# AlainSchoebi/semantic-bundle-adjustment-colmap

Measured on AMD Instinct MI355X. Metric: residuals+Jacobians/sec and BA-iteration wall-time, 1k cams / 1M pts / 10M obs, higher is better.
Workload: dtype f64

## Files before the change

semantic-bundle-adjustment-colmap_amd/csrc/context.h:

```cpp
#pragma once

#include <hip/hip_runtime.h>
#include <rocblas/rocblas.h>
#include <rccl/rccl.h>

#include <map>
#include <string>
#include <vector>

#include "../../include/mi_ba.h"
#include "cholesky.h"
#include "device.h"
#include "setup.h"

namespace miba {

template <typename T>
struct DevArray {
  T* ptr = nullptr;
  size_t n = 0;
  size_t cap = 0;
  DevArray() = default;
  DevArray(const DevArray&) = delete;
  DevArray& operator=(const DevArray&) = delete;
// ... 67 lines not shown
  int lin_overlap = 0;
  int lin_warm = 15;
  int lin_warm_conc = 0;
  int warm_unroll = 4;
  int warm_wgs = 2048;
  int lin_order = 0;
  int lin_fusion = 1;
  hipStream_t lin_side = nullptr;
  hipEvent_t lin_ev[2] = {nullptr, nullptr};
  int sem_diag = 0;
  bool sem_deferred_box = false;
  int sem_prep_early = 0;
  int sem_dgrid = 24;
  bool sem_dgrid_set = false;
  int sem_dwaves = 4;
  int sem_dvar = 0;
  int sem_compact = 1;
  int sem_coarse = 2;
  int sem_variant = 6;

  miba::DevArray<double2> r;
  miba::DevArray<double> J;
  miba::DevArray<double> Jcm;
  bool jcm_stale = true;
  miba::DevArray<double> Vg;
  miba::DevArray<double> partial;
  int64_t npartial = 0;
  miba::DevArray<double> scale_p, diag_p, Vinv;
  miba::DevArray<double> pose_blk, cam_blk, bvec, udiag;
  miba::DevArray<double> scale_f, diag_f, lambda_f, prec_pose, prec_cam;
// ... 84 lines not shown
```

semantic-bundle-adjustment-colmap_amd/csrc/runtime.hip:

```cpp
#include <hip/hip_runtime.h>

#include <algorithm>
#include <atomic>
#include <chrono>
#include <condition_variable>
#include <memory>
#include <mutex>
#include <thread>
#include <cmath>
#include <cstdio>
#include <cstring>
#include <cstdlib>
#include <map>
#include <numeric>
#include <unordered_map>

#include "../../include/mi_ba.h"
#include "ba_math.h"
#include "cholesky.h"
#include "context.h"
#include "kernels.h"
#include "gsba.h"
#include "semantic.h"
#include "setup.h"
// ... 2117 lines not shown
    return MI_BA_OK;
  }
  if (std::strcmp(key, "semantic_prep_early") == 0 && (value == 0 || value == 1) && ab_value(value, 0)) {
    ctx->sem_prep_early = value;
    return MI_BA_OK;
  }
  if (std::strcmp(key, "semantic_deferred_variant") == 0 && value >= 0 && value <= 4 && ab_value(value, 0)) {
    ctx->sem_dvar = value;
    return MI_BA_OK;
  }
  if (std::strcmp(key, "semantic_deferred_grid") == 0 && value >= 1 && value <= 64) {
    ctx->sem_dgrid = value;
    ctx->sem_dgrid_set = true;
    return MI_BA_OK;
  }
  if (std::strcmp(key, "semantic_deferred_waves") == 0 && (value == 1 || value == 4)) {
    ctx->sem_dwaves = value;
    return MI_BA_OK;
  }
  if (std::strcmp(key, "linearize_fusion") == 0 && value >= 0 && value <= 7) {
    ctx->lin_fusion = value;
    return MI_BA_OK;
  }
  if (std::strcmp(key, "semantic_deferred_compact") == 0 && (value == 0 || value == 1)) {
    ctx->sem_compact = value;
    return MI_BA_OK;
  }
  if (std::strcmp(key, "semantic_flat_coarse") == 0 && value >= 0 && value <= 3) {
    ctx->sem_coarse = value;
    return MI_BA_OK;
// ... 334 lines not shown
```

semantic-bundle-adjustment-colmap_amd/csrc/semantic.h:

```cpp
#pragma once

#include <hip/hip_runtime.h>

#include <cstdint>
#include <functional>

#include "../../include/mi_ba.h"
#include "ba_math.h"
#include "context.h"

namespace miba {

struct SemSample {
  double pc1[3];
  float label1;
  uint32_t pair;
};

struct SemTile {
  uint32_t pair, start, count, pad;
};

struct SemPair {
  uint32_t i, j;
// ... 35 lines not shown
  DevArray<double> r;
  DevArray<int32_t> status;
  DevArray<double> J;
  DevArray<double> pconst;
  bool samples_valid = false;
  DevArray<double> pair_blk;
  DevArray<double> partial;
  int64_t npartial = 0;
  DevArray<SemTile> tiles;
  int ntiles = 0;
  int model_tiles[kNumModels + 1] = {};
  DevArray<uint32_t> pair_cnt;
  DevArray<uint32_t> dlist;
  DevArray<uint2> chunks;
  DevArray<uint2> dchunks;
  DevArray<uint32_t> dcount;
  DevArray<uint32_t> model_pairs;
  DevArray<uint4> pair_ord;
  bool order_compact = false;
  int n_cu = 256;
  int dwaves_blocks[kNumModels] = {};
  int model_chunks[kNumModels + 1] = {};
  DevArray<unsigned long long> dmask;
  DevArray<uint32_t> pair_tile0, pair_chunk0;
  DevArray<double> cpart;
  DevArray<uint32_t> img_pairs_off, img_pairs;
  DevArray<uint2> sblk;
  DevArray<uint32_t> sblk_off, sblk_ent;
  int nsblk = 0;
  DevArray<double> mpart;
};

mi_ba_status semantic_create(mi_ba_context* ctx, const mi_ba_semantic* sem);
void semantic_destroy(mi_ba_context* ctx);
mi_ba_status semantic_linearize(mi_ba_context* ctx, double* d_cost, bool write_samples,
                                hipStream_t deferred_stream = nullptr, hipEvent_t flat_done = nullptr,
// ... 21 lines not shown
```

semantic-bundle-adjustment-colmap_amd/csrc/semantic.hip:

```cpp
#include <hip/hip_runtime.h>

#include <map>

#include <algorithm>
#include <cmath>
#include <cstring>
#include <type_traits>

#include "ba_math.h"
#include "kernels.h"
#include "semantic.h"
#include "step_bodies.h"

namespace miba {

namespace {

constexpr double kMinStep = 1.4901161193847656e-08;

struct SemArgs {
  const SemSample* samples;
  const SemPair* pairs;
  const double* qt;
  const double* cam;
// ... 310 lines not shown
  const int m = e >> 1;
  const bool minus = e & 1;
  const int grp = m < 4 ? 0 : (m < 7 ? 1 : (m < 11 ? 2 : 3));
  const int k = m - (grp == 0 ? 0 : (grp == 1 ? 4 : (grp == 2 ? 7 : 11)));
  const double orig = grp == 0 ? q1[k] : (grp == 1 ? t1[k] : (grp == 2 ? q2[k] : t2[k]));
  const double delta = fmax(kMinStep, fabs(orig) * rel_step);
  const double pert = minus ? orig - delta : orig + delta;
  P->pert[e] = pert;
  if (minus) {
    double one_over_delta = 1.0 / delta;
    one_over_delta /= 2;
    P->ood[m] = one_over_delta;
  }
  if (grp == 1 || grp == 3) return;
  const double* q = grp == 0 ? q1 : q2;
  double qq[4] = {q[0], q[1], q[2], q[3]};
  qq[k] = pert;
  double Q[9];
  quat_matrix_un(qq, Q);
  const double in = 1.0 / (qq[0] * qq[0] + qq[1] * qq[1] + qq[2] * qq[2] + qq[3] * qq[3]);
  double* A = P->A[grp == 0 ? e : e - 6];
  if (grp == 0) {
    double u2[4], R2[9];
    unit_quat(q2, u2);
    unit_quat_matrix(u2, R2);
    for (int r = 0; r < 3; ++r)
      for (int j = 0; j < 3; ++j)
        A[3 * r + j] = (R2[3 * r] * Q[3 * j] + R2[3 * r + 1] * Q[3 * j + 1] + R2[3 * r + 2] * Q[3 * j + 2]) * in;
  } else {
    for (int c = 0; c < 9; ++c) A[c] = Q[c] * in;
  }
  if (minus) {
    double PJ[12];
    quat_plus_jacobian(q, PJ);
    for (int c = 0; c < 3; ++c) P->pj[(grp == 0 ? 0 : 4) + k][c] = PJ[3 * k + c];
  }
}

constexpr int kPairVals = 78 + 12;
constexpr int kPairStride = 96;
constexpr int kSemRow = 13;

__device__ inline void pair_prep_body(int k, int lane, const SemPair* __restrict__ pairs, int npairs,
                                      const double* __restrict__ qt, const double* __restrict__ cam,
                                      const uint32_t* __restrict__ img_cam, const uint32_t* __restrict__ img_flags,
                                      const uint32_t* __restrict__ raster_slot, const SlotInfo* __restrict__ slots,
                                      double rel_step, PairConst* __restrict__ out, double* __restrict__ pair_blk,
                                      int blk_stride, uint32_t* __restrict__ pair_cnt) {
  if (k >= npairs) return;
  for (int e = lane; e < blk_stride; e += 32) pair_blk[(size_t)k * blk_stride + e] = 0.0;
  if (pair_cnt && lane == 31) pair_cnt[k] = 0u;
  if (lane > 28) return;
  const SemPair pr = pairs[k];
  if (lane < 28) {
    const double* a1 = qt + 8 * (size_t)pr.i;
    const double* a2 = qt + 8 * (size_t)pr.j;
    const double q1[4] = {a1[0], a1[1], a1[2], a1[3]}, t1[3] = {a1[4], a1[5], a1[6]};
    const double q2[4] = {a2[0], a2[1], a2[2], a2[3]}, t2[3] = {a2[4], a2[5], a2[6]};
    stencil_prep(q1, t1, q2, t2, rel_step, lane, out + k);
    return;
  }
  PairConst& P = out[k];
  const double* a1 = qt + 8 * (size_t)pr.i;
  const double* a2 = qt + 8 * (size_t)pr.j;
  for (int m = 0; m < 4; ++m) { P.q1[m] = a1[m]; P.q2[m] = a2[m]; }
  for (int m = 0; m < 3; ++m) { P.t1[m] = a1[4 + m]; P.t2[m] = a2[4 + m]; }
  Pose1Stage s;
  const double zero[3] = {0.0, 0.0, 0.0};
  pose1_stage(P.q1, zero, s);
  {
    const double* q1 = P.q1;
    const double sc = 1.0 / sqrt(q1[0] * q1[0] + q1[1] * q1[1] + q1[2] * q1[2] + q1[3] * q1[3]);
    const double qi[4] = {sc * q1[0], -(sc * q1[1]), -(sc * q1[2]), -(sc * q1[3])};
    const double scale = 1.0 / sqrt(qi[0] * qi[0] + qi[1] * qi[1] + qi[2] * qi[2] + qi[3] * qi[3]);
    for (int m = 0; m < 4; ++m) P.uqi[m] = scale * qi[m];
  }
  P.ti[0] = -(s.R[0] * P.t1[0] + s.R[1] * P.t1[1] + s.R[2] * P.t1[2]);
  P.ti[1] = -(s.R[3] * P.t1[0] + s.R[4] * P.t1[1] + s.R[5] * P.t1[2]);
  P.ti[2] = -(s.R[6] * P.t1[0] + s.R[7] * P.t1[1] + s.R[8] * P.t1[2]);
  unit_quat(P.q2, P.u2);
  unit_quat_matrix(P.u2, P.R2);
  for (int r = 0; r < 3; ++r)
    for (int c = 0; c < 3; ++c)
      P.C[3 * r + c] = P.R2[3 * r] * s.R[c] + P.R2[3 * r + 1] * s.R[3 + c] + P.R2[3 * r + 2] * s.R[6 + c];
  const double* K = cam + 8 * (size_t)img_cam[pr.j];
  for (int m = 0; m < 8; ++m) P.K2[m] = K[m];
  P.var1 = pr.var1;
  P.var2 = pr.var2;
  P.mask1 = (img_flags[pr.i] >> 1) & 7u;
  P.mask2 = (img_flags[pr.j] >> 1) & 7u;
  P.slot = raster_slot[pr.j];
  const SlotInfo si = slots[P.slot];
  P.H2 = (uint32_t)si.H;
  P.W2 = (uint32_t)si.W;
  P.TW2 = (uint32_t)si.TW;
  P.roff = si.off;
  P.toff = si.toff;
  stencil_bounds(P.q1, P.t1, rel_step, &P.rho1, P.dt1);
  stencil_bounds(P.q2, P.t2, rel_step, &P.rho2, P.dt2);
}

__global__ void semantic_pair_prep_kernel(const SemPair* __restrict__ pairs, int npairs, const double* __restrict__ qt,
                                          const double* __restrict__ cam, const uint32_t* __restrict__ img_cam,
                                          const uint32_t* __restrict__ img_flags,
                                          const uint32_t* __restrict__ raster_slot,
                                          const SlotInfo* __restrict__ slots, double rel_step,
                                          PairConst* __restrict__ out, double* __restrict__ pair_blk, int blk_stride,
                                          uint32_t* __restrict__ pair_cnt, uint32_t* __restrict__ zero_n = nullptr,
                                          int nzero = 0) {
  if (zero_n && blockIdx.x == 0 && (int)threadIdx.x < nzero) zero_n[threadIdx.x] = 0u;
  pair_prep_body(blockIdx.x * 2 + (threadIdx.x >> 5), threadIdx.x & 31, pairs, npairs, qt, cam, img_cam, img_flags,
                 raster_slot, slots, rel_step, out, pair_blk, blk_stride, pair_cnt);
}

// ... 2 lines not shown
  int npairs;
  const double* qt;
  const double* cam;
  const uint32_t* img_cam;
  const uint32_t* img_flags;
  const uint32_t* raster_slot;
  const SlotInfo* slots;
  double rel_step;
  PairConst* out;
  double* pair_blk;
  uint32_t* pair_cnt;
  uint32_t* dcount;
};

template <int U>
__global__ __launch_bounds__(256) void step_prologue_kernel(PrepArgs a, int nprep, DevProblem p,
                                                            double* __restrict__ rec, double* __restrict__ zero,
                                                            int nzero, int npack, TouchRanges t, unsigned* sink,
                                                            int nwarm) {
  const int b = blockIdx.x;
  if (b < nprep) {
    if (b == 0 && (int)threadIdx.x < kNumModels) a.dcount[threadIdx.x] = 0u;
    pair_prep_body(b * 8 + (threadIdx.x >> 5), threadIdx.x & 31, a.pairs, a.npairs, a.qt, a.cam, a.img_cam,
                   a.img_flags, a.raster_slot, a.slots, a.rel_step, a.out, a.pair_blk, kPairStride, a.pair_cnt);
  } else if (b < nprep + npack) {
    pack_image_record(p, rec, zero, nzero, (b - nprep) * 256 + (int)threadIdx.x);
  } else {
    touch_ranges<U>(t, sink, b - nprep - npack, nwarm);
  }
}

// ... 1119 lines not shown
    const double jm = (f2[0] - f2[1]) * P->ood[m];
    if constexpr (GRP == 0 || GRP == 2) {
      const double* pj = P->pj[(GRP == 0 ? 0 : 4) + k];
#pragma unroll
      for (int q = 0; q < 3; ++q) col[q] = col[q] + jm * pj[q];
    } else {
      const double v = ((mask >> k) & 1u) ? 0.0 : jm;
#pragma unroll
      for (int q = 0; q < 3; ++q) col[q] = q == k ? v : col[q];
    }
  }
  return true;
}

template <int M>
__global__ __launch_bounds__(256) void semantic_deferred_waves_kernel(SemArgs ak, const uint2* __restrict__ chunks,
                                                                     const uint32_t* __restrict__ ccount,
                                                                     const PairConst* __restrict__ pcs,
                                                                     const uint32_t* __restrict__ pair_cnt,
                                                                     const uint32_t* __restrict__ dlist,
                                                                     const uint32_t* __restrict__ pair_chunk0,
                                                                     double* __restrict__ cpart,
                                                                     double* __restrict__ J_out, int write_samples,
                                                                     int32_t* __restrict__ status_out = nullptr) {
  __shared__ double sraw[64 * 12];
  __shared__ double ssc[64], srs[64];
  __shared__ double sJ[64 * kSemRow];
  __shared__ uint8_t sredo[4 * 64];
  const int tid = threadIdx.x, lane = tid & 63;
  const int wv = __builtin_amdgcn_readfirstlane(tid >> 6);
  const uint32_t nch = ccount ? *ccount : blockIdx.x + 1;
  const uint32_t stride = ccount ? gridDim.x : 1u;
  for (uint32_t ci = blockIdx.x; ci < nch; ci += stride) {
    const uint2 ch = chunks[ci];
    const uint32_t cnt = pair_cnt[ch.x];
    if (ch.y >= cnt) continue;
    const PairConst* __restrict__ P = pcs + ch.x;
    const SemArgs a = with_pair(ak, P);
    const uint32_t k = ch.y + lane;
    const uint32_t pstart = a.pairs[ch.x].start;
    const float2* dl2 = a.dl + P->roff;
    const double* K2 = P->K2;
    double col[3] = {0.0, 0.0, 0.0};
    bool redone = false;
    int64_t n = 0;
    if (k < cnt) {
      n = (int64_t)pstart + dlist[pstart + k];
      const SemSample smp = a.samples[n];
      Centre c;
      if (wv == 0) {
        centre_geometry<M>(P, smp, K2, c);
        if (P->var1) redone = stencil_group<M, 0>(a, P, c, smp, K2, dl2, col);
      } else if (wv == 1) {
        centre_geometry<M>(P, smp, K2, c);
        if (P->var1) redone = stencil_group<M, 1>(a, P, c, smp, K2, dl2, col);
      } else if (wv == 2) {
        centre_geometry<M>(P, smp, K2, c);
        if (P->var2) redone = stencil_group<M, 2>(a, P, c, smp, K2, dl2, col);
      } else {
        centre_eval<M, true>(a, P, smp, K2, dl2, c);
        if (P->var2) redone = stencil_group<M, 3>(a, P, c, smp, K2, dl2, col);
        double rho[3];
        loss_eval(a.loss_type, a.loss_scale, c.r * c.r, rho);
        const double sc = sqrt(a.weight * rho[1]);
        ssc[lane] = sc;
        srs[lane] = c.r * sc;
      }
    }
#pragma unroll
    for (int q = 0; q < 3; ++q) sraw[lane * 12 + 3 * wv + q] = col[q];
    sredo[wv * 64 + lane] = redone ? 1 : 0;
    __syncthreads();
    if (tid < 64) {
      double rowv[kSemRow];
#pragma unroll
      for (int q = 0; q < kSemRow; ++q) rowv[q] = 0.0;
      if (k < cnt) {
        double Jt[12];
#pragma unroll
        for (int m = 0; m < 12; ++m) Jt[m] = sraw[lane * 12 + m];
        if ((write_samples & 4) && status_out && (sredo[lane] | sredo[64 + lane] | sredo[128 + lane] | sredo[192 + lane]))
          status_out[n] += 0x10000;
        if (write_samples) {
          double2* jo = reinterpret_cast<double2*>(J_out + 12 * n);
#pragma unroll
          for (int m = 0; m < 6; ++m) jo[m] = make_double2(Jt[2 * m], Jt[2 * m + 1]);
        }
        const double sc = ssc[lane];
#pragma unroll
        for (int m = 0; m < 12; ++m) rowv[m] = Jt[m] * sc;
        rowv[12] = srs[lane];
      }
#pragma unroll
      for (int q = 0; q < kSemRow; ++q) sJ[lane * kSemRow + q] = rowv[q];
    }
    __syncthreads();
    const int rows = min(64, (int)(cnt - ch.y));
    if (tid < kPairVals) {
      const int e = tid;
      int ca, cb;
      if (e < 78) {
        int a_ = 0, rem = e;
        while (rem >= 12 - a_) { rem -= 12 - a_; ++a_; }
        ca = a_;
        cb = a_ + rem;
      } else {
        ca = e - 78;
        cb = 12;
      }
      double acc = 0.0;
      for (int q = 0; q < rows; ++q) acc += sJ[q * kSemRow + ca] * sJ[q * kSemRow + cb];
      cpart[((size_t)pair_chunk0[ch.x] + ch.y / 64) * kPairVals + e] = acc;
    }
  }
}

template <bool COMPACT>
__global__ __launch_bounds__(256) void deferred_order_kernel(const unsigned long long* __restrict__ dmask,
                                                             const uint32_t* __restrict__ pair_tile0,
                                                             const SemPair* __restrict__ pairs,
                                                             uint32_t* __restrict__ pair_cnt,
                                                             uint32_t* __restrict__ dlist,
                                                             const uint4* __restrict__ ord = nullptr,
                                                             const uint32_t* __restrict__ mlist = nullptr,
                                                             uint2* __restrict__ dchunks = nullptr,
                                                             uint32_t* __restrict__ dcount = nullptr) {
  __shared__ uint32_t sc[256];
  __shared__ uint32_t spre[4];
  const int p = blockIdx.x, tid = threadIdx.x;
  const SemPair pr = pairs[p];
  const uint32_t words = (pr.count + 63) / 64;
  const unsigned long long* mk = dmask + (size_t)pair_tile0[p] * (kBlock / 64);
  uint4 od = make_uint4(0u, 0u, 0u, 0u);
  if constexpr (COMPACT) {
    od = ord[p];
    uint32_t pre = 0;
    for (uint32_t q = od.x + tid; q < od.y; q += 256) pre += (pair_cnt[mlist[q]] + 63) / 64;
    for (int off = 32; off > 0; off >>= 1) pre += __shfl_xor(pre, off, 64);
    if ((tid & 63) == 0) spre[tid >> 6] = pre;
  }
  uint32_t base = 0;
// ... 8 lines not shown
      __syncthreads();
      sc[tid] += v;
      __syncthreads();
    }
    uint32_t o = base + sc[tid] - c;
    for (unsigned long long r = m; r; r &= r - 1) dlist[pr.start + o++] = 64 * w + (uint32_t)__ffsll((long long)r) - 1;
    base += sc[255];
    __syncthreads();
  }
  if constexpr (COMPACT) {
    __syncthreads();
    const uint32_t pre = ((spre[0] + spre[1]) + spre[2]) + spre[3];
    const uint32_t nch = (base + 63) / 64;
    uint2* out = dchunks + od.w + pre;
    for (uint32_t c = tid; c < nch; c += 256) out[c] = make_uint2((uint32_t)p, 64 * c);
    if (tid == 0 && (od.z >> 31)) dcount[od.z & 0x7fffffffu] = pre + nch;
  } else {
    if (tid == 0) pair_cnt[p] = base;
  }
}

__global__ __launch_bounds__(128) void pair_reduce_kernel(const uint32_t* __restrict__ pair_cnt,
                                                          const uint32_t* __restrict__ pair_chunk0,
                                                          const double* __restrict__ cpart,
                                                          double* __restrict__ pair_blk) {
  pair_block_value(pair_cnt, pair_chunk0, cpart, pair_blk, kPairVals, kPairStride, blockIdx.x, threadIdx.x);
}

struct ModelRanges {
  int b[kNumModels + 1];
};

constexpr int kOrderCompactMaxPairs = 4096;

__global__ __launch_bounds__(256) void deferred_compact_kernel(const uint2* __restrict__ chunks, int nchunks,
                                                               const uint32_t* __restrict__ pair_cnt, ModelRanges mr,
                                                               uint2* __restrict__ out, uint32_t* __restrict__ cnt) {
  __shared__ uint32_t swc[4][kNumModels];
  __shared__ uint32_t sbase[kNumModels];
  const int i = blockIdx.x * 256 + threadIdx.x;
  const int lane = threadIdx.x & 63, wv = threadIdx.x >> 6;
  const bool valid = i < nchunks;
  uint2 ch = make_uint2(0u, 0u);
  int m = 0;
  bool live = false;
  if (valid) {
    ch = chunks[i];
    live = ch.y < pair_cnt[ch.x];
    while (m + 1 < kNumModels && i >= mr.b[m + 1]) ++m;
  }
  uint32_t rank = 0;
#pragma unroll
  for (int mm = 0; mm < kNumModels; ++mm) {
    const unsigned long long sel = __ballot(live && m == mm);
    if (lane == 0) swc[wv][mm] = (uint32_t)__popcll(sel);
    if (live && m == mm) rank = (uint32_t)__popcll(sel & ((1ull << lane) - 1ull));
  }
  __syncthreads();
  if (threadIdx.x < kNumModels) {
    const uint32_t tot = swc[0][threadIdx.x] + swc[1][threadIdx.x] + swc[2][threadIdx.x] + swc[3][threadIdx.x];
    sbase[threadIdx.x] = tot ? atomicAdd(cnt + threadIdx.x, tot) : 0u;
  }
  __syncthreads();
  if (live) {
    uint32_t off = sbase[m];
    for (int w = 0; w < wv; ++w) off += swc[w][m];
    out[mr.b[m] + off + rank] = ch;
  }
}

template <int M>
__global__ __launch_bounds__(kBlock) void semantic_cost_kernel(SemArgs a, double* __restrict__ partial) {
  __shared__ double sred[4];
  const int64_t n = (int64_t)blockIdx.x * kBlock + threadIdx.x;
  double c = 0.0;
  if (n < a.ns) {
    const SemSample smp = a.samples[n];
    const SemPair pr = a.pairs[smp.pair];
    const double* qt1 = a.qt + 8 * (size_t)pr.i;
    const double* qt2 = a.qt + 8 * (size_t)pr.j;
    const double q1[4] = {qt1[0], qt1[1], qt1[2], qt1[3]}, t1[3] = {qt1[4], qt1[5], qt1[6]};
    const double q2[4] = {qt2[0], qt2[1], qt2[2], qt2[3]}, t2[3] = {qt2[4], qt2[5], qt2[6]};
// ... 427 lines not shown
      if (per[m].size() > (size_t)kOrderCompactMaxPairs) S->order_compact = false;
      for (size_t r = 0; r < per[m].size(); ++r) {
        const uint32_t last = r + 1 == per[m].size() ? 0x80000000u : 0u;
        ord[per[m][r]] = make_uint4(begin, begin + (uint32_t)r, (uint32_t)m | last, (uint32_t)S->model_chunks[m]);
      }
      mlist.insert(mlist.end(), per[m].begin(), per[m].end());
    }
    if (S->pair_ord.alloc(ord.size()) || S->model_pairs.alloc(std::max<size_t>(1, mlist.size())))
      return MI_BA_ERR_OUT_OF_MEMORY;
    if (hipMemcpy(S->pair_ord.ptr, ord.data(), ord.size() * sizeof(uint4), hipMemcpyHostToDevice) ||
        (!mlist.empty() && hipMemcpy(S->model_pairs.ptr, mlist.data(), mlist.size() * 4, hipMemcpyHostToDevice)))
      return MI_BA_ERR_HIP;
  }
  if (S->pair_cnt.alloc(std::max(1, S->npairs)) || S->dlist.alloc(std::max<int64_t>(1, S->ns)) ||
      S->chunks.alloc(std::max<size_t>(1, chunks.size())) || S->dchunks.alloc(std::max<size_t>(1, chunks.size())) ||
      S->dcount.alloc(kNumModels))
    return MI_BA_ERR_OUT_OF_MEMORY;
  {
    const int np = S->npairs;
    std::vector<uint32_t> tile0(std::max(1, np), 0), chunk0(std::max(1, np), 0);
    for (size_t k = tiles.size(); k-- > 0;) tile0[tiles[k].pair] = (uint32_t)k;
    std::vector<uint32_t> nchk(std::max(1, np), 0);
    for (const uint2& c : chunks) ++nchk[c.x];
    for (size_t k = chunks.size(); k-- > 0;) chunk0[chunks[k].x] = (uint32_t)k;
    for (int k = 0; k < np; ++k) {
      const SemPair& pr = S->pairs_host[k];
      const uint32_t nt = (pr.count + kBlock - 1) / kBlock;
      for (uint32_t j = 0; j < nt; ++j)
        if (tiles[tile0[k] + j].pair != (uint32_t)k || tiles[tile0[k] + j].start != pr.start + j * kBlock)
          return MI_BA_ERR_HIP;
// ... 49 lines not shown
  }
  {
    int dev = 0, ncu = 0;
    if (hipGetDevice(&dev) != hipSuccess || hipDeviceGetAttribute(&ncu, hipDeviceAttributeMultiprocessorCount, dev) ||
        ncu <= 0)
      ncu = 256;
    S->n_cu = ncu;
    for (int model = 0; model < kNumModels; ++model) {
      dispatch_model(model, [&](auto m) {
        constexpr int M = decltype(m)::value;
        int nb = 0;
        if (hipOccupancyMaxActiveBlocksPerMultiprocessor(&nb, semantic_deferred_waves_kernel<M>, 256, 0) !=
                hipSuccess ||
            nb <= 0)
          nb = 4;
        S->dwaves_blocks[model] = nb;
      });
    }
  }
  if (!chunks.empty() && hipMemcpy(S->chunks.ptr, chunks.data(), chunks.size() * sizeof(uint2), hipMemcpyHostToDevice))
    return MI_BA_ERR_HIP;
  if (S->samples.alloc(S->ns) || S->pairs.alloc(S->npairs) || S->raster_slot.alloc(I) ||
      S->slots.alloc(std::max<size_t>(1, S->slots_host.size())) ||
      S->dl.alloc(std::max<size_t>(1, (size_t)S->npix)) || S->r.alloc(S->ns) ||
      S->status.alloc(S->ns) || S->J.alloc(12 * S->ns) ||
      S->pair_blk.alloc((size_t)kPairStride * std::max(1, S->npairs)) || S->tiles.alloc(tiles.size()) ||
      S->pconst.alloc(sizeof(PairConst) / sizeof(double) * std::max(1, S->npairs)))
    return MI_BA_ERR_OUT_OF_MEMORY;
  S->npartial = std::max<int64_t>({(int64_t)tiles.size(), (S->ns + kBlock - 1) / kBlock, (int64_t)1});
  if (S->partial.alloc(S->npartial)) return MI_BA_ERR_OUT_OF_MEMORY;
  if ((S->ns && hipMemcpy(S->samples.ptr, samples.data(), S->ns * sizeof(SemSample), hipMemcpyHostToDevice)) ||
// ... 192 lines not shown
  hipEvent_t stop;
  timer_begin_after(ctx, "semantic_jacobian", timer_start, &stop);
  const bool order_compact = (fusion & 2) && ctx->sem_variant == 6 && ctx->sem_compact != 0 && S->order_compact &&
                             S->model_chunks[kNumModels] > 0 && !deferred_stream;
  const bool epilogue = (fusion & 4) && ctx->sem_variant == 6 && other_partial && !deferred_stream;
  if (fusion & 1) {
  } else if (prep_done) {
    if (hipStreamWaitEvent(s, prep_done, 0) != hipSuccess) return MI_BA_ERR_HIP;
  } else {
    const mi_ba_status st = semantic_pair_prep(ctx, s);
    if (st != MI_BA_OK) return st;
  }
  const bool split = deferred_stream != nullptr && ctx->sem_variant == 6;
  if (ctx->sem_variant == 6) {
    const int ws = write_samples ? 1 | (ctx->sem_diag ? 2 : 0) | (ctx->sem_diag == 2 ? 4 : 0) : 0;
    auto deferred = [&](hipStream_t ds) -> mi_ba_status {
      if (order_compact)
        hipLaunchKernelGGL(deferred_order_kernel<true>, dim3(S->npairs), dim3(256), 0, ds, S->dmask.ptr,
                           S->pair_tile0.ptr, S->pairs.ptr, S->pair_cnt.ptr, S->dlist.ptr, S->pair_ord.ptr,
                           S->model_pairs.ptr, S->dchunks.ptr, S->dcount.ptr);
      else
        hipLaunchKernelGGL(deferred_order_kernel<false>, dim3(S->npairs), dim3(256), 0, ds, S->dmask.ptr,
                           S->pair_tile0.ptr, S->pairs.ptr, S->pair_cnt.ptr, S->dlist.ptr);
      const int nall = S->model_chunks[kNumModels];
      const bool compact = ctx->sem_compact != 0;
      if (nall > 0 && compact && !order_compact) {
        ModelRanges mr;
        for (int m = 0; m <= kNumModels; ++m) mr.b[m] = S->model_chunks[m];
        hipLaunchKernelGGL(deferred_compact_kernel, dim3((unsigned)((nall + 255) / 256)), dim3(256), 0, ds,
                           S->chunks.ptr, nall, S->pair_cnt.ptr, mr, S->dchunks.ptr, S->dcount.ptr);
      }
      for (int model = 0; model < kNumModels; ++model) {
        const int c0 = S->model_chunks[model], nc = S->model_chunks[model + 1] - c0;
        if (S->model_tiles[model + 1] == S->model_tiles[model] || nc == 0) continue;
        const bool waves4 = ctx->sem_dwaves == 4 && !ctx->sem_deferred_box
#ifdef MI_BA_AB_VARIANTS
                            && ctx->sem_dvar == 0
#endif
            ;
        const int per_cu = waves4 && !ctx->sem_dgrid_set ? std::max(1, S->dwaves_blocks[model])
                                                         : std::max(1, ctx->sem_dgrid);
        const int grid = compact ? std::min(nc, per_cu * S->n_cu) : nc;
        const uint2* list = (compact ? S->dchunks.ptr : S->chunks.ptr) + c0;
        const uint32_t* count = compact ? S->dcount.ptr + model : nullptr;
        dispatch_model(model, [&](auto m) {
          constexpr int M = decltype(m)::value;
          if (waves4)
            hipLaunchKernelGGL((semantic_deferred_waves_kernel<M>), dim3(grid), dim3(256), 0, ds, a, list, count,
                               pcs, S->pair_cnt.ptr, S->dlist.ptr, S->pair_chunk0.ptr, S->cpart.ptr, S->J.ptr, ws,
                               S->status.ptr);
          else if (ctx->sem_deferred_box)
            hipLaunchKernelGGL((semantic_deferred_kernel<M, true, 4, true>), dim3(grid), dim3(64), 0, ds, a, list,
                               count, pcs, S->pair_cnt.ptr, S->dlist.ptr, S->pair_chunk0.ptr, S->cpart.ptr, S->J.ptr,
                               ws, S->status.ptr);
#ifdef MI_BA_AB_VARIANTS
          else if (ctx->sem_dvar == 1)
            hipLaunchKernelGGL((semantic_deferred_kernel<M, true, 2>), dim3(grid), dim3(64), 0, ds, a, list, count,
                               pcs, S->pair_cnt.ptr, S->dlist.ptr, S->pair_chunk0.ptr, S->cpart.ptr, S->J.ptr, ws,
                               S->status.ptr);
          else if (ctx->sem_dvar == 2)
            hipLaunchKernelGGL((semantic_deferred_kernel<M, true, 2, false, 5>), dim3(grid), dim3(64), 0, ds, a,
                               list, count, pcs, S->pair_cnt.ptr, S->dlist.ptr, S->pair_chunk0.ptr, S->cpart.ptr, S->J.ptr,
// ... 164 lines not shown
```

semantic-bundle-adjustment-colmap_amd/csrc/step_bodies.h:

```cpp
#pragma once

#include <hip/hip_runtime.h>

#include <cstdint>

#include "device.h"

namespace miba {

__device__ inline void unit_quat_matrix_contracted(const double q[4], double R[9]) {
#pragma clang fp contract(fast)
  const double t2 = q[0] * q[1], t3 = q[0] * q[2], t4 = q[0] * q[3];
  const double t5 = -(q[1] * q[1]), t6 = q[1] * q[2], t7 = q[1] * q[3];
  const double t8 = -(q[2] * q[2]), t9 = q[2] * q[3], t1 = -(q[3] * q[3]);
  R[0] = 2.0 * (t8 + t1) + 1.0; R[1] = 2.0 * (t6 - t4);       R[2] = 2.0 * (t3 + t7);
  R[3] = 2.0 * (t4 + t6);       R[4] = 2.0 * (t5 + t1) + 1.0; R[5] = 2.0 * (t9 - t2);
  R[6] = 2.0 * (t7 - t3);       R[7] = 2.0 * (t2 + t9);       R[8] = 2.0 * (t5 + t8) + 1.0;
}

__device__ inline void pack_image_record(const DevProblem& p, double* __restrict__ rec, double* __restrict__ zero,
                                         int nzero, int k) {
#pragma clang fp contract(fast)
  if (k < nzero) zero[k] = 0.0;
  if (k >= p.num_images) return;
  const uint32_t cam = p.img_cam[k];
  double* o = rec + kImgRec * (size_t)k;
#pragma unroll
  for (int m = 0; m < 7; ++m) o[m] = p.qt[8 * (size_t)k + m];
  o[7] = __longlong_as_double(
      (long long)(p.img_flags[k] | ((p.cam_var[cam] != 0 ? 1u : 0u) << 8) | ((uint32_t)p.cam_model[cam] << 16)));
#pragma unroll
  for (int m = 0; m < 8; ++m) o[8 + m] = p.cam[8 * (size_t)cam + m];
  const double q[4] = {o[0], o[1], o[2], o[3]};
  double R[9];
  unit_quat_matrix_contracted(q, R);
#pragma unroll
  for (int m = 0; m < 9; ++m) o[16 + m] = R[m];
  o[25] = fabs(q[0] * q[0] + q[1] * q[1] + q[2] * q[2] + q[3] * q[3] - 1.0) <= 1e-12 ? 1.0 : 0.0;
#pragma unroll
  for (int m = 26; m < kImgRec; ++m) o[m] = 0.0;
}

struct TouchRanges {
  const uint4* ptr[5];
  int64_t n16[5];
};

template <int U>
__device__ inline void touch_ranges(const TouchRanges& t, unsigned* sink, int block, int nblocks) {
  unsigned acc = 0u;
  const int64_t stride = (int64_t)nblocks * 256;
#pragma unroll
  for (int q = 0; q < 5; ++q) {
    const uint4* a = t.ptr[q];
    const int64_t n = t.n16[q];
// ... 26 lines not shown
```

Before: 19.72 billion.

## Add software-pipelined deferred semantic kernel and split pair prep across lanes

Adds an optional pipelined path for the deferred waves kernel that prefetches chunk records, dlist entries and samples several iterations ahead. It uses a new per-chunk extent array (count, start) written by the order and compact kernels. The pair-prep body now spreads the pose-1, pose-2 and composed-rotation work across three lanes instead of one, and some unrolled selects replace dynamic indexing. Also adds a launch-bounds occupancy hint on the prologue and reorders the camera copy in image-record packing. The pipelined path is off by default; the pair-prep, launch-bounds and select changes are always on.

```diff
diff --git a/semantic-bundle-adjustment-colmap_amd/csrc/context.h b/semantic-bundle-adjustment-colmap_amd/csrc/context.h
--- a/semantic-bundle-adjustment-colmap_amd/csrc/context.h
+++ b/semantic-bundle-adjustment-colmap_amd/csrc/context.h
@@ -105,6 +105,8 @@
   int sem_dgrid = 24;
   bool sem_dgrid_set = false;
   int sem_dwaves = 4;
+  int sem_dpipe = 0;
+  int sem_dgroups = 0;
   int sem_dvar = 0;
   int sem_compact = 1;
   int sem_coarse = 2;
diff --git a/semantic-bundle-adjustment-colmap_amd/csrc/runtime.hip b/semantic-bundle-adjustment-colmap_amd/csrc/runtime.hip
--- a/semantic-bundle-adjustment-colmap_amd/csrc/runtime.hip
+++ b/semantic-bundle-adjustment-colmap_amd/csrc/runtime.hip
@@ -2155,6 +2155,14 @@
     ctx->sem_dgrid_set = true;
     return MI_BA_OK;
   }
+  if (std::strcmp(key, "semantic_deferred_pipeline") == 0 && (value == 0 || value == 1)) {
+    ctx->sem_dpipe = value;
+    return MI_BA_OK;
+  }
+  if (std::strcmp(key, "semantic_deferred_groups") == 0 && value >= 0 && value <= (1 << 20)) {
+    ctx->sem_dgroups = value;
+    return MI_BA_OK;
+  }
   if (std::strcmp(key, "semantic_deferred_waves") == 0 && (value == 1 || value == 4)) {
     ctx->sem_dwaves = value;
     return MI_BA_OK;
diff --git a/semantic-bundle-adjustment-colmap_amd/csrc/semantic.h b/semantic-bundle-adjustment-colmap_amd/csrc/semantic.h
--- a/semantic-bundle-adjustment-colmap_amd/csrc/semantic.h
+++ b/semantic-bundle-adjustment-colmap_amd/csrc/semantic.h
@@ -73,12 +73,13 @@
   DevArray<uint32_t> dlist;
   DevArray<uint2> chunks;
   DevArray<uint2> dchunks;
+  DevArray<uint2> dext;
   DevArray<uint32_t> dcount;
   DevArray<uint32_t> model_pairs;
   DevArray<uint4> pair_ord;
   bool order_compact = false;
   int n_cu = 256;
-  int dwaves_blocks[kNumModels] = {};
+  int dwaves_blocks[2][kNumModels] = {};
   int model_chunks[kNumModels + 1] = {};
   DevArray<unsigned long long> dmask;
   DevArray<uint32_t> pair_tile0, pair_chunk0;
diff --git a/semantic-bundle-adjustment-colmap_amd/csrc/semantic.hip b/semantic-bundle-adjustment-colmap_amd/csrc/semantic.hip
--- a/semantic-bundle-adjustment-colmap_amd/csrc/semantic.hip
+++ b/semantic-bundle-adjustment-colmap_amd/csrc/semantic.hip
@@ -348,8 +348,9 @@
   }
   if (grp == 1 || grp == 3) return;
   const double* q = grp == 0 ? q1 : q2;
-  double qq[4] = {q[0], q[1], q[2], q[3]};
-  qq[k] = pert;
+  double qq[4];
+#pragma unroll
+  for (int c = 0; c < 4; ++c) qq[c] = c == k ? pert : q[c];
   double Q[9];
   quat_matrix_un(qq, Q);
   const double in = 1.0 / (qq[0] * qq[0] + qq[1] * qq[1] + qq[2] * qq[2] + qq[3] * qq[3]);
@@ -367,7 +368,13 @@
   if (minus) {
     double PJ[12];
     quat_plus_jacobian(q, PJ);
-    for (int c = 0; c < 3; ++c) P->pj[(grp == 0 ? 0 : 4) + k][c] = PJ[3 * k + c];
+#pragma unroll
+    for (int c = 0; c < 3; ++c) {
+      double v = PJ[c];
+#pragma unroll
+      for (int kk = 1; kk < 4; ++kk) v = kk == k ? PJ[3 * kk + c] : v;
+      P->pj[(grp == 0 ? 0 : 4) + k][c] = v;
+    }
   }
 }
 
@@ -375,7 +382,7 @@
 constexpr int kPairStride = 96;
 constexpr int kSemRow = 13;
 
-__device__ inline void pair_prep_body(int k, int lane, const SemPair* __restrict__ pairs, int npairs,
+__device__ __forceinline__ void pair_prep_body(int k, int lane, const SemPair* __restrict__ pairs, int npairs,
                                       const double* __restrict__ qt, const double* __restrict__ cam,
                                       const uint32_t* __restrict__ img_cam, const uint32_t* __restrict__ img_flags,
                                       const uint32_t* __restrict__ raster_slot, const SlotInfo* __restrict__ slots,
@@ -384,54 +391,67 @@
   if (k >= npairs) return;
   for (int e = lane; e < blk_stride; e += 32) pair_blk[(size_t)k * blk_stride + e] = 0.0;
   if (pair_cnt && lane == 31) pair_cnt[k] = 0u;
-  if (lane > 28) return;
+  if (lane > 30) return;
   const SemPair pr = pairs[k];
-  if (lane < 28) {
-    const double* a1 = qt + 8 * (size_t)pr.i;
-    const double* a2 = qt + 8 * (size_t)pr.j;
-    const double q1[4] = {a1[0], a1[1], a1[2], a1[3]}, t1[3] = {a1[4], a1[5], a1[6]};
-    const double q2[4] = {a2[0], a2[1], a2[2], a2[3]}, t2[3] = {a2[4], a2[5], a2[6]};
-    stencil_prep(q1, t1, q2, t2, rel_step, lane, out + k);
-    return;
-  }
-  PairConst& P = out[k];
   const double* a1 = qt + 8 * (size_t)pr.i;
   const double* a2 = qt + 8 * (size_t)pr.j;
-  for (int m = 0; m < 4; ++m) { P.q1[m] = a1[m]; P.q2[m] = a2[m]; }
-  for (int m = 0; m < 3; ++m) { P.t1[m] = a1[4 + m]; P.t2[m] = a2[4 + m]; }
-  Pose1Stage s;
+  if (lane < 28) {
+    stencil_prep(a1, a1 + 4, a2, a2 + 4, rel_step, lane, out + k);
+    return;
+  }
+  PairConst& P = out[k];
   const double zero[3] = {0.0, 0.0, 0.0};
-  pose1_stage(P.q1, zero, s);
-  {
-    const double* q1 = P.q1;
-    const double sc = 1.0 / sqrt(q1[0] * q1[0] + q1[1] * q1[1] + q1[2] * q1[2] + q1[3] * q1[3]);
-    const double qi[4] = {sc * q1[0], -(sc * q1[1]), -(sc * q1[2]), -(sc * q1[3])};
-    const double scale = 1.0 / sqrt(qi[0] * qi[0] + qi[1] * qi[1] + qi[2] * qi[2] + qi[3] * qi[3]);
-    for (int m = 0; m < 4; ++m) P.uqi[m] = scale * qi[m];
-  }
-  P.ti[0] = -(s.R[0] * P.t1[0] + s.R[1] * P.t1[1] + s.R[2] * P.t1[2]);
-  P.ti[1] = -(s.R[3] * P.t1[0] + s.R[4] * P.t1[1] + s.R[5] * P.t1[2]);
-  P.ti[2] = -(s.R[6] * P.t1[0] + s.R[7] * P.t1[1] + s.R[8] * P.t1[2]);
-  unit_quat(P.q2, P.u2);
-  unit_quat_matrix(P.u2, P.R2);
-  for (int r = 0; r < 3; ++r)
-    for (int c = 0; c < 3; ++c)
-      P.C[3 * r + c] = P.R2[3 * r] * s.R[c] + P.R2[3 * r + 1] * s.R[3 + c] + P.R2[3 * r + 2] * s.R[6 + c];
-  const double* K = cam + 8 * (size_t)img_cam[pr.j];
-  for (int m = 0; m < 8; ++m) P.K2[m] = K[m];
-  P.var1 = pr.var1;
-  P.var2 = pr.var2;
-  P.mask1 = (img_flags[pr.i] >> 1) & 7u;
-  P.mask2 = (img_flags[pr.j] >> 1) & 7u;
-  P.slot = raster_slot[pr.j];
-  const SlotInfo si = slots[P.slot];
-  P.H2 = (uint32_t)si.H;
-  P.W2 = (uint32_t)si.W;
-  P.TW2 = (uint32_t)si.TW;
-  P.roff = si.off;
-  P.toff = si.toff;
-  stencil_bounds(P.q1, P.t1, rel_step, &P.rho1, P.dt1);
-  stencil_bounds(P.q2, P.t2, rel_step, &P.rho2, P.dt2);
+  if (lane == 28) {
+    const double q1[4] = {a1[0], a1[1], a1[2], a1[3]}, t1[3] = {a1[4], a1[5], a1[6]};
+    for (int m = 0; m < 4; ++m) P.q1[m] = q1[m];
+    for (int m = 0; m < 3; ++m) P.t1[m] = t1[m];
+    Pose1Stage s;
+    pose1_stage(q1, zero, s);
+    {
+      const double sc = 1.0 / sqrt(q1[0] * q1[0] + q1[1] * q1[1] + q1[2] * q1[2] + q1[3] * q1[3]);
+      const double qi[4] = {sc * q1[0], -(sc * q1[1]), -(sc * q1[2]), -(sc * q1[3])};
+      const double scale = 1.0 / sqrt(qi[0] * qi[0] + qi[1] * qi[1] + qi[2] * qi[2] + qi[3] * qi[3]);
+      for (int m = 0; m < 4; ++m) P.uqi[m] = scale * qi[m];
+    }
+    P.ti[0] = -(s.R[0] * t1[0] + s.R[1] * t1[1] + s.R[2] * t1[2]);
+    P.ti[1] = -(s.R[3] * t1[0] + s.R[4] * t1[1] + s.R[5] * t1[2]);
+    P.ti[2] = -(s.R[6] * t1[0] + s.R[7] * t1[1] + s.R[8] * t1[2]);
+    P.var1 = pr.var1;
+    P.mask1 = (img_flags[pr.i] >> 1) & 7u;
+    stencil_bounds(q1, t1, rel_step, &P.rho1, P.dt1);
+  } else if (lane == 29) {
+    const double q2[4] = {a2[0], a2[1], a2[2], a2[3]}, t2[3] = {a2[4], a2[5], a2[6]};
+    for (int m = 0; m < 4; ++m) P.q2[m] = q2[m];
+    for (int m = 0; m < 3; ++m) P.t2[m] = t2[m];
+    double u2[4], R2[9];
+    unit_quat(q2, u2);
+    unit_quat_matrix(u2, R2);
+    for (int m = 0; m < 4; ++m) P.u2[m] = u2[m];
+    for (int m = 0; m < 9; ++m) P.R2[m] = R2[m];
+    const double* K = cam + 8 * (size_t)img_cam[pr.j];
+    for (int m = 0; m < 8; ++m) P.K2[m] = K[m];
+    P.var2 = pr.var2;
+    P.mask2 = (img_flags[pr.j] >> 1) & 7u;
+    const uint32_t slot = raster_slot[pr.j];
+    P.slot = slot;
+    const SlotInfo si = slots[slot];
+    P.H2 = (uint32_t)si.H;
+    P.W2 = (uint32_t)si.W;
+    P.TW2 = (uint32_t)si.TW;
+    P.roff = si.off;
+    P.toff = si.toff;
+    stencil_bounds(q2, t2, rel_step, &P.rho2, P.dt2);
+  } else {
+    const double q1[4] = {a1[0], a1[1], a1[2], a1[3]}, q2[4] = {a2[0], a2[1], a2[2], a2[3]};
+    Pose1Stage s;
+    pose1_stage(q1, zero, s);
+    double u2[4], R2[9];
+    unit_quat(q2, u2);
+    unit_quat_matrix(u2, R2);
+    for (int r = 0; r < 3; ++r)
+      for (int c = 0; c < 3; ++c)
+        P.C[3 * r + c] = R2[3 * r] * s.R[c] + R2[3 * r + 1] * s.R[3 + c] + R2[3 * r + 2] * s.R[6 + c];
+  }
 }
 
 __global__ void semantic_pair_prep_kernel(const SemPair* __restrict__ pairs, int npairs, const double* __restrict__ qt,
@@ -464,7 +484,7 @@
 };
 
 template <int U>
-__global__ __launch_bounds__(256) void step_prologue_kernel(PrepArgs a, int nprep, DevProblem p,
+__global__ __launch_bounds__(256, 8) void step_prologue_kernel(PrepArgs a, int nprep, DevProblem p,
                                                             double* __restrict__ rec, double* __restrict__ zero,
                                                             int nzero, int npack, TouchRanges t, unsigned* sink,
                                                             int nwarm) {
@@ -1614,6 +1634,90 @@
 }
 
 template <int M>
+__device__ __forceinline__ void deferred_waves_chunk(const SemArgs& ak, const PairConst* __restrict__ pcs,
+                                                     const uint32_t* __restrict__ pair_chunk0,
+                                                     double* __restrict__ cpart, double* __restrict__ J_out,
+                                                     int write_samples, int32_t* __restrict__ status_out,
+                                                     double* sraw, double* ssc, double* srs, double* sJ,
+                                                     uint8_t* sredo, int tid, int lane, int wv, uint2 ch,
+                                                     uint32_t cnt, int64_t n, const SemSample& smp) {
+  if (ch.y >= cnt) return;
+  const PairConst* __restrict__ P = pcs + ch.x;
+  const SemArgs a = with_pair(ak, P);
+  const uint32_t k = ch.y + lane;
+  const float2* dl2 = a.dl + P->roff;
+  const double* K2 = P->K2;
+  double col[3] = {0.0, 0.0, 0.0};
+  bool redone = false;
+  if (k < cnt) {
+    Centre c;
+    if (wv == 0) {
+      centre_geometry<M>(P, smp, K2, c);
+      if (P->var1) redone = stencil_group<M, 0>(a, P, c, smp, K2, dl2, col);
+    } else if (wv == 1) {
+      centre_geometry<M>(P, smp, K2, c);
+      if (P->var1) redone = stencil_group<M, 1>(a, P, c, smp, K2, dl2, col);
+    } else if (wv == 2) {
+      centre_geometry<M>(P, smp, K2, c);
+      if (P->var2) redone = stencil_group<M, 2>(a, P, c, smp, K2, dl2, col);
+    } else {
+      centre_eval<M, true>(a, P, smp, K2, dl2, c);
+      if (P->var2) redone = stencil_group<M, 3>(a, P, c, smp, K2, dl2, col);
+      double rho[3];
+      loss_eval(a.loss_type, a.loss_scale, c.r * c.r, rho);
+      const double sc = sqrt(a.weight * rho[1]);
+      ssc[lane] = sc;
+      srs[lane] = c.r * sc;
+    }
+  }
+#pragma unroll
+  for (int q = 0; q < 3; ++q) sraw[lane * 12 + 3 * wv + q] = col[q];
+  sredo[wv * 64 + lane] = redone ? 1 : 0;
+  __syncthreads();
+  if (tid < 64) {
+    double rowv[kSemRow];
+#pragma unroll
+    for (int q = 0; q < kSemRow; ++q) rowv[q] = 0.0;
+    if (k < cnt) {
+      double Jt[12];
+#pragma unroll
+      for (int m = 0; m < 12; ++m) Jt[m] = sraw[lane * 12 + m];
+      if ((write_samples & 4) && status_out && (sredo[lane] | sredo[64 + lane] | sredo[128 + lane] | sredo[192 + lane]))
+        status_out[n] += 0x10000;
+      if (write_samples) {
+        double2* jo = reinterpret_cast<double2*>(J_out + 12 * n);
+#pragma unroll
+        for (int m = 0; m < 6; ++m) jo[m] = make_double2(Jt[2 * m], Jt[2 * m + 1]);
+      }
+      const double sc = ssc[lane];
+#pragma unroll
+      for (int m = 0; m < 12; ++m) rowv[m] = Jt[m] * sc;
+      rowv[12] = srs[lane];
+    }
+#pragma unroll
+    for (int q = 0; q < kSemRow; ++q) sJ[lane * kSemRow + q] = rowv[q];
+  }
+  __syncthreads();
+  const int rows = min(64, (int)(cnt - ch.y));
+  if (tid < kPairVals) {
+    const int e = tid;
+    int ca, cb;
+    if (e < 78) {
+      int a_ = 0, rem = e;
+      while (rem >= 12 - a_) { rem -= 12 - a_; ++a_; }
+      ca = a_;
+      cb = a_ + rem;
+    } else {
+      ca = e - 78;
+      cb = 12;
+    }
+    double acc = 0.0;
+    for (int q = 0; q < rows; ++q) acc += sJ[q * kSemRow + ca] * sJ[q * kSemRow + cb];
+    cpart[((size_t)pair_chunk0[ch.x] + ch.y / 64) * kPairVals + e] = acc;
+  }
+}
+
+template <int M, bool PIPE = false>
 __global__ __launch_bounds__(256) void semantic_deferred_waves_kernel(SemArgs ak, const uint2* __restrict__ chunks,
                                                                      const uint32_t* __restrict__ ccount,
                                                                      const PairConst* __restrict__ pcs,
@@ -1622,7 +1726,8 @@
                                                                      const uint32_t* __restrict__ pair_chunk0,
                                                                      double* __restrict__ cpart,
                                                                      double* __restrict__ J_out, int write_samples,
-                                                                     int32_t* __restrict__ status_out = nullptr) {
+                                                                     int32_t* __restrict__ status_out = nullptr,
+                                                                     const uint2* __restrict__ cext = nullptr) {
   __shared__ double sraw[64 * 12];
   __shared__ double ssc[64], srs[64];
   __shared__ double sJ[64 * kSemRow];
@@ -1631,86 +1736,56 @@
   const int wv = __builtin_amdgcn_readfirstlane(tid >> 6);
   const uint32_t nch = ccount ? *ccount : blockIdx.x + 1;
   const uint32_t stride = ccount ? gridDim.x : 1u;
-  for (uint32_t ci = blockIdx.x; ci < nch; ci += stride) {
-    const uint2 ch = chunks[ci];
-    const uint32_t cnt = pair_cnt[ch.x];
-    if (ch.y >= cnt) continue;
-    const PairConst* __restrict__ P = pcs + ch.x;
-    const SemArgs a = with_pair(ak, P);
-    const uint32_t k = ch.y + lane;
-    const uint32_t pstart = a.pairs[ch.x].start;
-    const float2* dl2 = a.dl + P->roff;
-    const double* K2 = P->K2;
-    double col[3] = {0.0, 0.0, 0.0};
-    bool redone = false;
-    int64_t n = 0;
-    if (k < cnt) {
-      n = (int64_t)pstart + dlist[pstart + k];
-      const SemSample smp = a.samples[n];
-      Centre c;
-      if (wv == 0) {
-        centre_geometry<M>(P, smp, K2, c);
-        if (P->var1) redone = stencil_group<M, 0>(a, P, c, smp, K2, dl2, col);
-      } else if (wv == 1) {
-        centre_geometry<M>(P, smp, K2, c);
-        if (P->var1) redone = stencil_group<M, 1>(a, P, c, smp, K2, dl2, col);
-      } else if (wv == 2) {
-        centre_geometry<M>(P, smp, K2, c);
-        if (P->var2) redone = stencil_group<M, 2>(a, P, c, smp, K2, dl2, col);
-      } else {
-        centre_eval<M, true>(a, P, smp, K2, dl2, c);
-        if (P->var2) redone = stencil_group<M, 3>(a, P, c, smp, K2, dl2, col);
-        double rho[3];
-        loss_eval(a.loss_type, a.loss_scale, c.r * c.r, rho);
-        const double sc = sqrt(a.weight * rho[1]);
-        ssc[lane] = sc;
-        srs[lane] = c.r * sc;
+  if constexpr (PIPE) {
+    const uint2 none = make_uint2(0u, 0u);
+    auto uniform = [](uint2 v) {
+      return make_uint2((uint32_t)__builtin_amdgcn_readfirstlane((int)v.x),
+                        (uint32_t)__builtin_amdgcn_readfirstlane((int)v.y));
+    };
+    auto record = [&](uint32_t c, uint2& ch, uint2& ex) {
+      ch = uniform(c < nch ? chunks[c] : none);
+      ex = uniform(c < nch ? cext[c] : none);
+    };
+    auto entry = [&](uint32_t c, uint2 ch, uint2 ex) -> uint32_t {
+      return c < nch && ch.y + lane < ex.x ? dlist[ex.y + ch.y + lane] : 0u;
+    };
+    auto sample = [&](uint32_t c, uint2 ch, uint2 ex, uint32_t e) -> SemSample {
+      SemSample smp = {{0.0, 0.0, 0.0}, 0.f, 0u};
+      if (c < nch && ch.y + lane < ex.x) smp = ak.samples[(int64_t)ex.y + e];
+      return smp;
+    };
+    uint32_t ci = blockIdx.x;
+    uint2 ch0, ex0, ch1, ex1, ch2, ex2;
+    record(ci, ch0, ex0);
+    record(ci + stride, ch1, ex1);
+    record(ci + 2 * stride, ch2, ex2);
+    uint32_t e0 = entry(ci, ch0, ex0), e1 = entry(ci + stride, ch1, ex1);
+    SemSample s0 = sample(ci, ch0, ex0, e0);
+    for (; ci < nch; ci += stride) {
+      uint2 ch3, ex3;
+      record(ci + 3 * stride, ch3, ex3);
+      const uint32_t e2 = entry(ci + 2 * stride, ch2, ex2);
+      const SemSample s1 = sample(ci + stride, ch1, ex1, e1);
+      deferred_waves_chunk<M>(ak, pcs, pair_chunk0, cpart, J_out, write_samples, status_out, sraw, ssc, srs, sJ, sredo,
+                              tid, lane, wv, ch0, ex0.x, (int64_t)ex0.y + e0, s0);
+      ch0 = ch1, ex0 = ex1, e0 = e1, s0 = s1;
+      ch1 = ch2, ex1 = ex2, e1 = e2;
+      ch2 = ch3, ex2 = ex3;
+    }
+  } else {
+    for (uint32_t ci = blockIdx.x; ci < nch; ci += stride) {
+      const uint2 ch = chunks[ci];
+      const uint32_t cnt = pair_cnt[ch.x];
+      if (ch.y >= cnt) continue;
+      const uint32_t pstart = ak.pairs[ch.x].start;
+      int64_t n = 0;
+      SemSample smp = {{0.0, 0.0, 0.0}, 0.f, 0u};
+      if (ch.y + lane < cnt) {
+        n = (int64_t)pstart + dlist[pstart + ch.y + lane];
+        smp = ak.samples[n];
       }
-    }
-#pragma unroll
-    for (int q = 0; q < 3; ++q) sraw[lane * 12 + 3 * wv + q] = col[q];
-    sredo[wv * 64 + lane] = redone ? 1 : 0;
-    __syncthreads();
-    if (tid < 64) {
-      double rowv[kSemRow];
-#pragma unroll
-      for (int q = 0; q < kSemRow; ++q) rowv[q] = 0.0;
-      if (k < cnt) {
-        double Jt[12];
-#pragma unroll
-        for (int m = 0; m < 12; ++m) Jt[m] = sraw[lane * 12 + m];
-        if ((write_samples & 4) && status_out && (sredo[lane] | sredo[64 + lane] | sredo[128 + lane] | sredo[192 + lane]))
-          status_out[n] += 0x10000;
-        if (write_samples) {
-          double2* jo = reinterpret_cast<double2*>(J_out + 12 * n);
-#pragma unroll
-          for (int m = 0; m < 6; ++m) jo[m] = make_double2(Jt[2 * m], Jt[2 * m + 1]);
-        }
-        const double sc = ssc[lane];
-#pragma unroll
-        for (int m = 0; m < 12; ++m) rowv[m] = Jt[m] * sc;
-        rowv[12] = srs[lane];
-      }
-#pragma unroll
-      for (int q = 0; q < kSemRow; ++q) sJ[lane * kSemRow + q] = rowv[q];
-    }
-    __syncthreads();
-    const int rows = min(64, (int)(cnt - ch.y));
-    if (tid < kPairVals) {
-      const int e = tid;
-      int ca, cb;
-      if (e < 78) {
-        int a_ = 0, rem = e;
-        while (rem >= 12 - a_) { rem -= 12 - a_; ++a_; }
-        ca = a_;
-        cb = a_ + rem;
-      } else {
-        ca = e - 78;
-        cb = 12;
-      }
-      double acc = 0.0;
-      for (int q = 0; q < rows; ++q) acc += sJ[q * kSemRow + ca] * sJ[q * kSemRow + cb];
-      cpart[((size_t)pair_chunk0[ch.x] + ch.y / 64) * kPairVals + e] = acc;
+      deferred_waves_chunk<M>(ak, pcs, pair_chunk0, cpart, J_out, write_samples, status_out, sraw, ssc, srs, sJ, sredo,
+                              tid, lane, wv, ch, cnt, n, smp);
     }
   }
 }
@@ -1724,7 +1799,8 @@
                                                              const uint4* __restrict__ ord = nullptr,
                                                              const uint32_t* __restrict__ mlist = nullptr,
                                                              uint2* __restrict__ dchunks = nullptr,
-                                                             uint32_t* __restrict__ dcount = nullptr) {
+                                                             uint32_t* __restrict__ dcount = nullptr,
+                                                             uint2* __restrict__ dext = nullptr) {
   __shared__ uint32_t sc[256];
   __shared__ uint32_t spre[4];
   const int p = blockIdx.x, tid = threadIdx.x;
@@ -1763,6 +1839,8 @@
     const uint32_t nch = (base + 63) / 64;
     uint2* out = dchunks + od.w + pre;
     for (uint32_t c = tid; c < nch; c += 256) out[c] = make_uint2((uint32_t)p, 64 * c);
+    if (dext)
+      for (uint32_t c = tid; c < nch; c += 256) dext[od.w + pre + c] = make_uint2(base, pr.start);
     if (tid == 0 && (od.z >> 31)) dcount[od.z & 0x7fffffffu] = pre + nch;
   } else {
     if (tid == 0) pair_cnt[p] = base;
@@ -1784,18 +1862,22 @@
 
 __global__ __launch_bounds__(256) void deferred_compact_kernel(const uint2* __restrict__ chunks, int nchunks,
                                                                const uint32_t* __restrict__ pair_cnt, ModelRanges mr,
-                                                               uint2* __restrict__ out, uint32_t* __restrict__ cnt) {
+                                                               uint2* __restrict__ out, uint32_t* __restrict__ cnt,
+                                                               const SemPair* __restrict__ pairs = nullptr,
+                                                               uint2* __restrict__ ext = nullptr) {
   __shared__ uint32_t swc[4][kNumModels];
   __shared__ uint32_t sbase[kNumModels];
   const int i = blockIdx.x * 256 + threadIdx.x;
   const int lane = threadIdx.x & 63, wv = threadIdx.x >> 6;
   const bool valid = i < nchunks;
   uint2 ch = make_uint2(0u, 0u);
+  uint32_t pcnt = 0;
   int m = 0;
   bool live = false;
   if (valid) {
     ch = chunks[i];
-    live = ch.y < pair_cnt[ch.x];
+    pcnt = pair_cnt[ch.x];
+    live = ch.y < pcnt;
     while (m + 1 < kNumModels && i >= mr.b[m + 1]) ++m;
   }
   uint32_t rank = 0;
@@ -1815,6 +1897,7 @@
     uint32_t off = sbase[m];
     for (int w = 0; w < wv; ++w) off += swc[w][m];
     out[mr.b[m] + off + rank] = ch;
+    if (ext) ext[mr.b[m] + off + rank] = make_uint2(pcnt, pairs[ch.x].start);
   }
 }
 
@@ -2272,6 +2355,7 @@
   }
   if (S->pair_cnt.alloc(std::max(1, S->npairs)) || S->dlist.alloc(std::max<int64_t>(1, S->ns)) ||
       S->chunks.alloc(std::max<size_t>(1, chunks.size())) || S->dchunks.alloc(std::max<size_t>(1, chunks.size())) ||
+      S->dext.alloc(std::max<size_t>(1, chunks.size())) ||
       S->dcount.alloc(kNumModels))
     return MI_BA_ERR_OUT_OF_MEMORY;
   {
@@ -2351,7 +2435,12 @@
                 hipSuccess ||
             nb <= 0)
           nb = 4;
-        S->dwaves_blocks[model] = nb;
+        S->dwaves_blocks[0][model] = nb;
+        if (hipOccupancyMaxActiveBlocksPerMultiprocessor(&nb, semantic_deferred_waves_kernel<M, true>, 256, 0) !=
+                hipSuccess ||
+            nb <= 0)
+          nb = 4;
+        S->dwaves_blocks[1][model] = nb;
       });
     }
   }
@@ -2574,11 +2663,17 @@
   const bool split = deferred_stream != nullptr && ctx->sem_variant == 6;
   if (ctx->sem_variant == 6) {
     const int ws = write_samples ? 1 | (ctx->sem_diag ? 2 : 0) | (ctx->sem_diag == 2 ? 4 : 0) : 0;
+    const bool pipe = ctx->sem_dpipe != 0 && ctx->sem_compact != 0 && ctx->sem_dwaves == 4 && !ctx->sem_deferred_box
+#ifdef MI_BA_AB_VARIANTS
+                      && ctx->sem_dvar == 0
+#endif
+        ;
+    uint2* dext = pipe ? S->dext.ptr : nullptr;
     auto deferred = [&](hipStream_t ds) -> mi_ba_status {
       if (order_compact)
         hipLaunchKernelGGL(deferred_order_kernel<true>, dim3(S->npairs), dim3(256), 0, ds, S->dmask.ptr,
                            S->pair_tile0.ptr, S->pairs.ptr, S->pair_cnt.ptr, S->dlist.ptr, S->pair_ord.ptr,
-                           S->model_pairs.ptr, S->dchunks.ptr, S->dcount.ptr);
+                           S->model_pairs.ptr, S->dchunks.ptr, S->dcount.ptr, dext);
       else
         hipLaunchKernelGGL(deferred_order_kernel<false>, dim3(S->npairs), dim3(256), 0, ds, S->dmask.ptr,
                            S->pair_tile0.ptr, S->pairs.ptr, S->pair_cnt.ptr, S->dlist.ptr);
@@ -2588,7 +2683,8 @@
         ModelRanges mr;
         for (int m = 0; m <= kNumModels; ++m) mr.b[m] = S->model_chunks[m];
         hipLaunchKernelGGL(deferred_compact_kernel, dim3((unsigned)((nall + 255) / 256)), dim3(256), 0, ds,
-                           S->chunks.ptr, nall, S->pair_cnt.ptr, mr, S->dchunks.ptr, S->dcount.ptr);
+                           S->chunks.ptr, nall, S->pair_cnt.ptr, mr, S->dchunks.ptr, S->dcount.ptr, S->pairs.ptr,
+                           dext);
       }
       for (int model = 0; model < kNumModels; ++model) {
         const int c0 = S->model_chunks[model], nc = S->model_chunks[model + 1] - c0;
@@ -2598,14 +2694,19 @@
                             && ctx->sem_dvar == 0
 #endif
             ;
-        const int per_cu = waves4 && !ctx->sem_dgrid_set ? std::max(1, S->dwaves_blocks[model])
+        const int per_cu = waves4 && !ctx->sem_dgrid_set ? std::max(1, S->dwaves_blocks[pipe ? 1 : 0][model])
                                                          : std::max(1, ctx->sem_dgrid);
-        const int grid = compact ? std::min(nc, per_cu * S->n_cu) : nc;
+        const int resident = ctx->sem_dgroups > 0 ? ctx->sem_dgroups : per_cu * S->n_cu;
+        const int grid = compact ? std::min(nc, resident) : nc;
         const uint2* list = (compact ? S->dchunks.ptr : S->chunks.ptr) + c0;
         const uint32_t* count = compact ? S->dcount.ptr + model : nullptr;
         dispatch_model(model, [&](auto m) {
           constexpr int M = decltype(m)::value;
-          if (waves4)
+          if (waves4 && pipe)
+            hipLaunchKernelGGL((semantic_deferred_waves_kernel<M, true>), dim3(grid), dim3(256), 0, ds, a, list, count,
+                               pcs, S->pair_cnt.ptr, S->dlist.ptr, S->pair_chunk0.ptr, S->cpart.ptr, S->J.ptr, ws,
+                               S->status.ptr, dext + c0);
+          else if (waves4)
             hipLaunchKernelGGL((semantic_deferred_waves_kernel<M>), dim3(grid), dim3(256), 0, ds, a, list, count,
                                pcs, S->pair_cnt.ptr, S->dlist.ptr, S->pair_chunk0.ptr, S->cpart.ptr, S->J.ptr, ws,
                                S->status.ptr);
diff --git a/semantic-bundle-adjustment-colmap_amd/csrc/step_bodies.h b/semantic-bundle-adjustment-colmap_amd/csrc/step_bodies.h
--- a/semantic-bundle-adjustment-colmap_amd/csrc/step_bodies.h
+++ b/semantic-bundle-adjustment-colmap_amd/csrc/step_bodies.h
@@ -29,8 +29,6 @@
   for (int m = 0; m < 7; ++m) o[m] = p.qt[8 * (size_t)k + m];
   o[7] = __longlong_as_double(
       (long long)(p.img_flags[k] | ((p.cam_var[cam] != 0 ? 1u : 0u) << 8) | ((uint32_t)p.cam_model[cam] << 16)));
-#pragma unroll
-  for (int m = 0; m < 8; ++m) o[8 + m] = p.cam[8 * (size_t)cam + m];
   const double q[4] = {o[0], o[1], o[2], o[3]};
   double R[9];
   unit_quat_matrix_contracted(q, R);
@@ -39,6 +37,8 @@
   o[25] = fabs(q[0] * q[0] + q[1] * q[1] + q[2] * q[2] + q[3] * q[3] - 1.0) <= 1e-12 ? 1.0 : 0.0;
 #pragma unroll
   for (int m = 26; m < kImgRec; ++m) o[m] = 0.0;
+#pragma unroll
+  for (int m = 0; m < 8; ++m) o[8 + m] = p.cam[8 * (size_t)cam + m];
 }
 
 struct TouchRanges {
```

Measured after the change: 20.06 billion (median of 6 runs). +1.8%, better.
